# AdrianoEttari/DiffusionRemoteSensing

Hardware: AMD Instinct MI355X
Metric: unet_denoise_steps_per_s (higher is better)
Workload: dtype f16 main + block-scaled fp6 (e2m3) cross terms of tap pairs on the wide 3x3 layers (FL, 11 of 11 launches of the dominant kernel); split bf16 x3 (hi + lo) everywhere else; f32 accumulate

## Files before the change

### diffusionremotesensing_amd/_lib.py

```python
import ctypes as C
import os

_HERE = os.path.dirname(os.path.abspath(__file__))
LIB_PATH = os.path.join(_HERE, "libdrs_hip.so")

IMPL_DIRECT, IMPL_MFMA_F32, IMPL_MFMA_BF16X3, IMPL_MFMA_F16 = 0, 1, 2, 3
IMPL_BY_NAME = {"direct": IMPL_DIRECT, "mfma_f32": IMPL_MFMA_F32, "mfma_bf16x3": IMPL_MFMA_BF16X3,
                "mfma_f16": IMPL_MFMA_F16}
FWD_REUSE_COND = 1
PLAN_KEEP_ALL = 1
PLAN_TRAIN = 2
VARIANT_SUPERRES, VARIANT_SAR_TO_NDVI, VARIANT_GENERATION = 0, 1, 2


class UNetConfig(C.Structure):
    _fields_ = [("batch", C.c_int), ("lr_batch", C.c_int), ("image_channels", C.c_int), ("out_dim", C.c_int),
                ("height", C.c_int), ("width", C.c_int), ("magnification", C.c_int), ("impl", C.c_int),
                ("bn_eps", C.c_float), ("flags", C.c_int), ("variant", C.c_int),
                ("cond_channels", C.c_int), ("num_classes", C.c_int)]


_P, _I, _L, _Z, _F = C.c_void_p, C.c_int, C.c_int64, C.c_size_t, C.c_float
SIGNATURES = {
    "drs_last_error": (C.c_char_p, []),
    "drs_abi_version": (_I, []),
    "drs_noise_images": (_I, [_P, _P, _P, _P, _I, _P, _I, _L, _P]),
    "drs_sampler_step": (_I, [_P, _P, _P, _I, _P, _P, _P, _I, _L, _P]),
    "drs_sampler_step_cfg": (_I, [_P, _P, _P, C.c_float, _P, _I, _P, _P, _P, _I, C.c_int64, _P]),
    "drs_ddim_step": (_I, [_P, _P, _P, C.c_float, _P, _I, _I, C.c_float, _P, _I, C.c_int64, _P]),
    "drs_inpaint_step": (_I, [_P, _P, _P, _F, _P, _P, _P] + [_I] * 8 + [_F, _P, _P, _P, _I, _P]),
    "drs_renoise": (_I, [_P, _P, _I, _I, _P, _I, _L, _P]),
    "drs_adam_multi": (_I, [_P, _I, C.c_int64, C.c_double, C.c_double, C.c_double, C.c_double, _P]),
    "drs_ema_multi": (_I, [_P, _I, C.c_int64, C.c_double, _I, _P]),
    "drs_downblur_scratch_bytes": (_Z, [_I, _I, _I, _I, _I, _I]),
    "drs_downblur_u8": (_I, [_P, _I, _I, _I, _I, _I, _I, C.c_float, _P, _P, _P, _Z, _P]),
    "drs_add_noise_clip_f32": (_I, [_P, _P, _I, _I, _I, _I, _P]),
    "drs_gather_pairs_f32": (_I, [_P, _P, _P, _I, _L, _I, _I, _P, _P, _P]),
    "drs_gather_u8_f32": (_I, [_P, _P, _P, _I, _L, _I, _P, _P, _P]),
    "drs_aggregate_tiles": (_I, [_P, _P, _P, _P, _P, _I, _I, _I, _I, _I, _P]),
    "drs_gather_tiles": (_I, [_P, _P, _P, _I, _I, _I, _I, _I, _I, _I, _P]),
    "drs_blend_step": (_I, [_P] * 6 + [_I] * 6 + [_P, _P, _P, _I, _P]),
    "drs_blend_step_ddim": (_I, [_P] * 6 + [_I] * 7 + [_F, _P, _I, _P]),
    "drs_metrics_workspace_bytes": (_Z, [_I] * 4),
    "drs_metrics_pointwise": (_I, [_P, _P, _P] + [_I] * 5 + [_P, _Z, _P]),
    "drs_ssim": (_I, [_P, _P, _P] + [_I] * 5 + [_P, _Z, _P]),
    "drs_conv2d_workspace_bytes": (_Z, [_I] * 11),
    "drs_conv2d_nchw": (_I, [_P, _P, _P, _P] + [_I] * 12 + [_P, _Z, _I, _P]),
    "drs_upconv_fused_workspace_bytes": (_Z, [_I] * 5),
    "drs_upconv_fused_nchw": (_I, [_P] * 9 + [_I] + [_P, _P] + [_I] * 5 + [_P, _Z, _P]),
    "drs_bicubic_upsample_nchw": (_I, [_P, _P, _I, _I, _I, _I, _I, _P]),
    "drs_time_mlp": (_I, [_P] * 7 + [_I, _I, _I, _P]),
    "drs_unet_plan_create": (_I, [C.POINTER(_P), C.POINTER(UNetConfig)]),
    "drs_unet_plan_destroy": (None, [_P]),
    "drs_unet_num_params": (_I, [_P]),
    "drs_unet_param_name": (C.c_char_p, [_P, _I]),
    "drs_unet_param_numel": (_L, [_P, _I]),
    "drs_unet_packed_bytes": (_Z, [_P]),
    "drs_unet_workspace_bytes": (_Z, [_P]),
    "drs_unet_pack_weights": (_I, [_P, C.POINTER(_P), C.POINTER(_F), _P, _Z, _P]),
    "drs_unet_forward": (_I, [_P, _P, _P, _P, _P, _P, _P, _Z, _I, _P]),
    "drs_unet_forward_labels": (_I, [_P, _P, _P, _P, _P, _P, _I, _P, _P, _Z, _I, _P]),
    "drs_unet_num_tensors": (_I, [_P]),
    "drs_unet_tensor_name": (C.c_char_p, [_P, _I]),
    "drs_unet_tensor_shape": (_I, [_P, _I] + [C.POINTER(_I)] * 4),
    "drs_unet_read_tensor": (_I, [_P, _I, _P, _P, _P]),
    "drs_unet_packed_bwd_bytes": (_Z, [_P]),
    "drs_unet_backward": (_I, [_P, _P, _P, _Z, _P, _P, _P, C.POINTER(_P), _P, _Z, _P]),
    "drs_unet_backward_labels": (_I, [_P, _P, _P, _Z, _P, _P, _P, _I, _P, C.POINTER(_P), _P, _Z, _P]),
    "drs_unet_check_faults": (_I, [_P, _P, _P]),
    "drs_unet_profile_enable": (_I, [_P, _I]),
    "drs_unet_profile_num_ops": (_I, [_P]),
    "drs_unet_profile_read": (_I, [_P, _I, C.c_char_p, _I, C.POINTER(_F), C.POINTER(C.c_double), C.POINTER(C.c_double)]),
    "drs_unet_profile_num_launches": (_I, [_P]),
    "drs_unet_profile_launch": (_I, [_P, _I, C.c_char_p, _I, C.c_char_p, _I]),
    "drs_vgg_plan_create": (_I, [C.POINTER(_P), _I, _I, _I, _I]),
    "drs_vgg_plan_destroy": (None, [_P]),
    "drs_vgg_packed_bytes": (_Z, [_P]),
    "drs_vgg_workspace_bytes": (_Z, [_P]),
    "drs_vgg_pack_weights": (_I, [_P, C.POINTER(_P), _P, _Z, _P]),
    "drs_vgg_forward": (_I, [_P, _P, _P, _P, _P, _I, _P, _Z, _P]),
    "drs_vgg_backward": (_I, [_P, _P, _P, _P, _P, _Z, _P]),
    "drs_vgg_profile_enable": (_I, [_P, _I]),
    "drs_vgg_profile_num_ops": (_I, [_P]),
    "drs_vgg_profile_read": (_I, [_P, _I, C.c_char_p, _I, C.POINTER(_F), C.POINTER(C.c_double)]),
}

_lib = None


def lib_path():
    return os.environ.get("DRS_LIB", LIB_PATH)


def load():
    global _lib
    if _lib is not None:
        return _lib
    path = lib_path()
    if not os.path.exists(path):
        raise RuntimeError(
            f"{path} not found: the HIP kernels are not built. Run `python -c 'import __graft_entry__ as g; "
            "g.build()'` (needs hipcc, cross-compiles for gfx950 without a GPU). There is no CPU fallback.")
    lib = C.CDLL(path)
    for name, (res, args) in SIGNATURES.items():
        fn = getattr(lib, name)
        fn.restype = res
        fn.argtypes = args
    _lib = lib
    return lib


class RangeFault(RuntimeError):
    """DRS_ERR_RANGE from drs_unet_check_faults: an activation left fp16's range in the FL arithmetic; the plan has switched
    itself to the split-bf16 kernels, the forwards since the last check must be run again."""


def check(status, what):
    if status != 0:
# ... 6 lines not shown
```

### diffusionremotesensing_amd/csrc/resblock0_sp.hip

```cpp
#include <stdio.h>
#include <stdlib.h>

#include "conv_epilogue.h"
#include "mfma_policy.h"
#include "sp_sync.h"

namespace {

constexpr int TW_ = 16, TH_ = 8, IW = TW_ + 2, IH = TH_ + 2, NPIX = IW * IH, NBLK_A = (NPIX + 15) / 16;
constexpr int IMG1 = 5 * 4 * 64 * 16, IMG2 = 36 * 32 * 16, IMGS = 4 * 32 * 16, WIN = NPIX * 128;
constexpr int NPOST = 16;
constexpr int XPLANE = (TH_ + 4) * (TW_ + 4) * 16 + 64, XT = 4 * XPLANE;

#ifdef DRS_SP_TIMELINE
__device__ unsigned long long drs_rb0_tl[32];
#define RB_STAMP(i) do { const unsigned long long t_ = __builtin_amdgcn_s_memtime(); tl[i] += t_ - tl_last; tl_last = t_; } while (0)
#else
#define RB_STAMP(i) do { } while (0)
#endif

__global__ __launch_bounds__(512, 1) void resblock0_kernel(ResBlock0Desc d, unsigned w1_gimage, unsigned w2_gimage,
                                                           unsigned ws_gimage, int debug) {
  extern __shared__ __attribute__((aligned(16))) char smem[];
  using P = PolicyBF16X3;
  using Frag = typename P::Frag;
  auto mfma = [](const bf16x8& w, const bf16x8& x, const f32x4& c) __attribute__((always_inline)) {
    return __builtin_amdgcn_mfma_f32_16x16x32_bf16(w, x, c, 0, 0, 0);
  };
  const int tid = threadIdx.x, lane = tid & 63, wave = __builtin_amdgcn_readfirstlane(tid >> 6);
  const int lr = lane & 15, kg = lane >> 4;
  char* sW1 = smem;
  char* sW2 = sW1 + 2 * IMG1;
  char* sWs = sW2 + 2 * IMG2;
  char* sWinAll = sWs + 2 * IMGS;
  char* sXAll = sWinAll + 2 * WIN;
  float* sB1 = reinterpret_cast<float*>(sXAll + 2 * XT);
  float* sB2 = sB1 + 64;
  unsigned* sCntRaw = reinterpret_cast<unsigned*>(sB2 + 32);
  float* sPost = sB2 + 32 + 8;
  const int npost = min(d.N, NPOST);
  {
    const char* w1 = reinterpret_cast<const char*>(d.w1);
    for (int i = tid; i < 2 * 20 * 64; i += 512) {
      const int im = i >= 20 * 64, idx = im ? i - 20 * 64 : i;
      const int ch = idx % 64, kgp = (idx / 64) & 3, j = idx / (4 * 64), tap = 2 * j + (kgp >> 1);
      u32x4 v = {0u, 0u, 0u, 0u};
      if (tap < 9) v = *reinterpret_cast<const u32x4*>(w1 + (size_t)im * w1_gimage + ((size_t)(tap * 4 + (kgp & 1)) * 64 + ch) * 16);
      *reinterpret_cast<u32x4*>(sW1 + (size_t)im * IMG1 + (size_t)idx * 16) = v;
    }
    auto copy = [&](char* dst, const char* src, int bytes) __attribute__((always_inline)) {
      for (int o = tid * 16; o < bytes; o += 512 * 16) *reinterpret_cast<u32x4*>(dst + o) = *reinterpret_cast<const u32x4*>(src + o);
    };
    const char* w2 = reinterpret_cast<const char*>(d.w2);
    const char* wsc = reinterpret_cast<const char*>(d.ws);
    copy(sW2, w2, IMG2);
    copy(sW2 + IMG2, w2 + w2_gimage, IMG2);
    copy(sWs, wsc, IMGS);
    copy(sWs + IMGS, wsc + ws_gimage, IMGS);
    for (int i = tid; i < 64; i += 512) sB1[i] = d.b1[i];
    for (int i = tid; i < 32; i += 512) sB2[i] = d.b2[i] + d.bs[i];
    if (tid < 8) sCntRaw[tid] = 0u;
    for (int i = tid; i < npost * 32; i += 512) sPost[i] = d.temb[(size_t)(i >> 5) * d.temb_cs + (i & 31)];
  }
  __syncthreads();

  const int grp = wave >> 2, gw = wave & 3;
  char* sWin = sWinAll + grp * WIN;
  const sp_flag_ptr cWritten = (sp_flag_ptr)(sCntRaw + 2 * grp), cRead = (sp_flag_ptr)(sCntRaw + 2 * grp + 1);
  const int gx = d.W / TW_, gy = d.H / TH_;
  const int total = d.N * gy * gx;
  const int xcd = blockIdx.x & 7, member = blockIdx.x >> 3, members = gridDim.x >> 3;
  const int t_lo = (int)((long long)total * xcd / 8), t_hi = (int)((long long)total * (xcd + 1) / 8);
  const char* zero = reinterpret_cast<const char*>(d.zero_line);
  const char* xb = reinterpret_cast<const char*>(d.x);
  char* sX = sXAll + grp * XT;
  const sp_flag_ptr cTile = (sp_flag_ptr)(sCntRaw + 4 + grp);
  constexpr int XPIX = (TH_ + 4) * (TW_ + 4), XW = TW_ + 4;
  int tx0 = 0, ty0 = 0, n = 0;
  const int qstep_ = 2 * (int)(gridDim.x >> 3);
  const int step_x = qstep_ % gx, step_y = (qstep_ / gx) % gy, step_n = qstep_ / (gx * gy);
  int bx = 0, by = 0;
  auto place_first = [&](int q) __attribute__((always_inline)) {
    bx = q % gx; by = (q / gx) % gy; n = q / (gx * gy);
    tx0 = bx * TW_; ty0 = by * TH_;
  };
  auto place_next = [&]() __attribute__((always_inline)) {
    bx += step_x;
    if (bx >= gx) { bx -= gx; ++by; }
    by += step_y;
    if (by >= gy) { by -= gy; ++n; }
    n += step_n;
    tx0 = bx * TW_; ty0 = by * TH_;
  };
  unsigned goff[4];
#pragma unroll
  for (int i = 0; i < 4; ++i) {
    const int e = i * 256 + gw * 64 + lane, pix = min(e >> 2, XPIX - 1);
    const int py = (pix * 3277) >> 16, px = pix - py * XW;
    goff[i] = (unsigned)((py * d.W + px) * 64 + (e & 3) * 16);
  }
  u32x4 xr[4];
  auto tile_load = [&]() __attribute__((always_inline)) {
    const char* ximg = xb + (size_t)n * d.H * d.W * 64;
    if (ty0 >= 2 && ty0 + TH_ + 2 <= d.H && tx0 >= 2 && tx0 + TW_ + 2 <= d.W) {
      typedef const __attribute__((address_space(1))) char* gptr;
      const unsigned long long gi = (unsigned long long)(ximg + ((long long)(ty0 - 2) * d.W + (tx0 - 2)) * 64);
      gptr g = (gptr)(((unsigned long long)(unsigned)__builtin_amdgcn_readfirstlane((int)(gi >> 32)) << 32) |
                      (unsigned)__builtin_amdgcn_readfirstlane((int)(unsigned)gi));
      asm volatile("" : "+s"(g));
#pragma unroll
      for (int i = 0; i < 4; ++i) xr[i] = *(const __attribute__((address_space(1))) u32x4*)(g + goff[i]);
    } else {
#pragma unroll
      for (int i = 0; i < 4; ++i) {
        const int e = i * 256 + gw * 64 + lane, pix = e >> 2;
        const int py = (pix * 3277) >> 16, px = pix - py * XW;
        const int y = ty0 - 2 + py, x = tx0 - 2 + px;
        const bool ok = pix < XPIX && y >= 0 && y < d.H && x >= 0 && x < d.W;
        xr[i] = *reinterpret_cast<const u32x4*>(ok ? ximg + ((size_t)y * d.W + x) * 64 + (e & 3) * 16 : zero);
      }
    }
  };
  auto tile_store = [&]() __attribute__((always_inline)) {
#pragma unroll
    for (int i = 0; i < 4; ++i) {
      const int e = i * 256 + gw * 64 + lane;
      if ((e >> 2) < XPIX) *reinterpret_cast<u32x4*>(sX + (e & 3) * XPLANE + (e >> 2) * 16) = xr[i];
    }
    sp_release(cTile, lane);
  };
  constexpr int MAXB = NBLK_A / 4;
  static_assert(MAXB * 4 == NBLK_A, "three blocks per wave");
  int wp[MAXB], relL[MAXB], tapL[5];
#pragma unroll
  for (int b = 0; b < MAXB; ++b) {
    const int p = min((gw + 4 * b) * 16 + lr, NPIX - 1);
    const int py = (p * 3641) >> 16, px = p - py * IW;
    wp[b] = p;
    relL[b] = ((py + 1) * XW + px + 1) * 16 + (kg & 1) * XPLANE;
  }
#pragma unroll
  for (int j = 0; j < 5; ++j) {
    const int tap = min(2 * j + (kg >> 1), 8);
    tapL[j] = ((tap / 3 - 1) * XW + tap % 3 - 1) * 16;
  }
  auto operand = [&](int b, int j) __attribute__((always_inline)) {
    const char* p = sX + relL[b] + tapL[j];
    return Frag{*reinterpret_cast<const bf16x8*>(p), *reinterpret_cast<const bf16x8*>(p + 2 * XPLANE)};
  };
  const int q0 = t_lo + 2 * member + grp, qstep = 2 * members;
#ifdef DRS_SP_TIMELINE
  unsigned long long tl[8] = {0, 0, 0, 0, 0, 0, 0, 0};
  const unsigned long long tl_begin = __builtin_amdgcn_s_memtime();
  unsigned long long tl_last = tl_begin, tl_n = 0;
  if ((debug & 1) && grp == 1) return;
#endif
  if (q0 < t_hi) {
    place_first(q0);
    tile_load();
    tile_store();
    if (q0 + qstep < t_hi) {
      place_next();
      tile_load();
      asm volatile("" :: "v"(xr[0]), "v"(xr[1]), "v"(xr[2]), "v"(xr[3]));
    }
  }
  if (grp == 1) { __builtin_amdgcn_s_sleep(64); __builtin_amdgcn_s_sleep(32); }
  unsigned k = 0;
  u32x4 kept[4] = {};
  int cbx = q0 % gx, cby = (q0 / gx) % gy, cn = q0 / (gx * gy);
  for (int q = q0; q < t_hi; q += qstep, ++k) {
#ifdef DRS_SP_TIMELINE
    ++tl_n;
#endif
    RB_STAMP(7);
    const int cty0 = cby * TH_, ctx0 = cbx * TW_;
    sp_poll_lds(cTile, 4u * (k + 1), d.fault);
    const bool more = q + qstep < t_hi;
    f32x4 acc[MAXB][4];
#pragma unroll
    for (int b = 0; b < MAXB; ++b)
#pragma unroll
      for (int t = 0; t < 4; ++t) acc[b][t] = f32x4{0.f, 0.f, 0.f, 0.f};
    const char* w1lane = sW1 + ((size_t)kg * 64 + lr) * 16;
    Frag a[2][MAXB], wfa[2][2];
#pragma unroll
    for (int b = 0; b < MAXB; ++b) a[0][b] = operand(b, 0);
#pragma unroll
    for (int u = 0; u < 2; ++u) wfa[0][u] = P::load(w1lane, (size_t)IMG1, (size_t)(u * 16) * 16);
#pragma unroll
    for (int st = 0; st < 10; ++st) {
      const int j = st >> 1, h = st & 1;
      if (st + 1 < 10) {
#pragma unroll
        for (int u = 0; u < 2; ++u)
          wfa[(st + 1) & 1][u] = P::load(w1lane, (size_t)IMG1, (size_t)(((st + 1) >> 1) * 4 * 64 + (((st + 1) & 1) * 2 + u) * 16) * 16);
      }
      if (h == 0 && j + 1 < 5) {
#pragma unroll
        for (int b = 0; b < MAXB; ++b) a[(j + 1) & 1][b] = operand(b, j + 1);
      }
      {
        const Frag (&wf)[2] = wfa[st & 1];
#pragma unroll
        for (int u = 0; u < 2; ++u)
#pragma unroll
          for (int b = 0; b < MAXB; ++b) acc[b][2 * h + u] = mfma(wf[u].lo, a[j & 1][b].hi, acc[b][2 * h + u]);
#pragma unroll
        for (int u = 0; u < 2; ++u)
#pragma unroll
          for (int b = 0; b < MAXB; ++b) acc[b][2 * h + u] = mfma(wf[u].hi, a[j & 1][b].lo, acc[b][2 * h + u]);
#pragma unroll
        for (int u = 0; u < 2; ++u)
#pragma unroll
          for (int b = 0; b < MAXB; ++b) acc[b][2 * h + u] = mfma(wf[u].hi, a[j & 1][b].hi, acc[b][2 * h + u]);
      }
      if (h == 0 && j + 1 < 5) __builtin_amdgcn_sched_group_barrier(0x100, 4 + 2 * MAXB, 0);
      else if (st + 1 < 10) __builtin_amdgcn_sched_group_barrier(0x100, 4, 0);
      __builtin_amdgcn_sched_group_barrier(0x008, 18, 0);
      __builtin_amdgcn_sched_barrier(0);
    }
    asm volatile("" :: "v"(kept[0]), "v"(kept[1]), "v"(kept[2]), "v"(kept[3]));
    RB_STAMP(0);
    Frag xs[2];
#pragma unroll
    for (int r = 0; r < 2; ++r) {
      const char* p = sX + ((2 + 2 * gw + r) * XW + 2 + lr) * 16 + (kg & 1) * XPLANE;
      xs[r] = Frag{*reinterpret_cast<const bf16x8*>(p), *reinterpret_cast<const bf16x8*>(p + 2 * XPLANE)};
    }
    float bm[8], bs[8], te[8];
    {
      const float4 m0 = *reinterpret_cast<const float4*>(sB1 + kg * 8), m1 = *reinterpret_cast<const float4*>(sB1 + kg * 8 + 4);
      const float4 s0 = *reinterpret_cast<const float4*>(sB1 + 32 + kg * 8), s1 = *reinterpret_cast<const float4*>(sB1 + 32 + kg * 8 + 4);
      float4 e0, e1;
      if (cn < npost) {
        e0 = *reinterpret_cast<const float4*>(sPost + cn * 32 + kg * 8); e1 = *reinterpret_cast<const float4*>(sPost + cn * 32 + kg * 8 + 4);
      } else {
        const float* gp = d.temb + (size_t)cn * d.temb_cs + kg * 8;
        e0 = *reinterpret_cast<const float4*>(gp); e1 = *reinterpret_cast<const float4*>(gp + 4);
      }
      bm[0] = m0.x; bm[1] = m0.y; bm[2] = m0.z; bm[3] = m0.w; bm[4] = m1.x; bm[5] = m1.y; bm[6] = m1.z; bm[7] = m1.w;
      bs[0] = s0.x; bs[1] = s0.y; bs[2] = s0.z; bs[3] = s0.w; bs[4] = s1.x; bs[5] = s1.y; bs[6] = s1.z; bs[7] = s1.w;
      te[0] = e0.x; te[1] = e0.y; te[2] = e0.z; te[3] = e0.w; te[4] = e1.x; te[5] = e1.y; te[6] = e1.z; te[7] = e1.w;
    }
    RB_STAMP(1);
    sp_poll_lds(cRead, 4u * k, d.fault);
    RB_STAMP(2);
#pragma unroll
    for (int b = 0; b < MAXB; ++b) {
      float v[8];
#pragma unroll
      for (int t = 0; t < 2; ++t)
#pragma unroll
        for (int i = 0; i < 4; ++i)
          v[t * 4 + i] = (drs_maxf(acc[b][t][i] + bm[t * 4 + i], 0.f) + (acc[b][t + 2][i] + bs[t * 4 + i])) + te[t * 4 + i];
      u32x4 hh, hl;
      drs_sp_split8(v, hh, hl);
      int p = wp[b];
      asm volatile("" : "+v"(p));
      const int py = (p * 3641) >> 16, px = p - py * IW;
      const int y = cty0 - 1 + py, x = ctx0 - 1 + px;
      const bool inside = y >= 0 && y < d.H && x >= 0 && x < d.W;
      if (!inside) { hh = u32x4{0u, 0u, 0u, 0u}; hl = u32x4{0u, 0u, 0u, 0u}; }
      if ((gw + 4 * b) * 16 + lr < NPIX) {
        char* wpix = sWin + p * 128;
        const int s0 = ((kg + p) & 7) * 16;
        *reinterpret_cast<u32x4*>(wpix + s0) = hh;
        *reinterpret_cast<u32x4*>(wpix + (s0 ^ 64)) = hl;
      }
    }
    sp_release(cWritten, lane);
    sp_poll_lds(cWritten, 4u * (k + 1), d.fault);
    if (more) tile_store();
    RB_STAMP(3);
    f32x4 o[2][2];
#pragma unroll
    for (int r = 0; r < 2; ++r)
#pragma unroll
      for (int t = 0; t < 2; ++t) o[r][t] = f32x4{0.f, 0.f, 0.f, 0.f};
    const char* w2lane = sW2 + ((size_t)kg * 32 + lr) * 16;
    auto win = [&](int row, int kx) __attribute__((always_inline)) {
      const int p = (2 * gw + row) * IW + lr + kx;
      const char* wpix = sWin + p * 128;
      const int s0 = ((kg + p) & 7) * 16;
      return Frag{*reinterpret_cast<const bf16x8*>(wpix + s0), *reinterpret_cast<const bf16x8*>(wpix + (s0 ^ 64))};
    };
    Frag wr_[4][3];
    auto win_row = [&](int row) __attribute__((always_inline)) {
#pragma unroll
      for (int kx = 0; kx < 3; ++kx) wr_[row][kx] = win(row, kx);
    };
    win_row(0);
    win_row(1);
    {
      const char* wslane = sWs + ((size_t)kg * 32 + lr) * 16;
      Frag wfb[2][2];
      wfb[0][0] = P::load(w2lane, (size_t)IMG2, 0);
      wfb[0][1] = P::load(w2lane, (size_t)IMG2, (size_t)16 * 16);
#pragma unroll
      for (int st = 0; st < 10; ++st) {
#pragma unroll
        for (int t = 0; t < 2; ++t) {
          if (st + 1 < 9) wfb[(st + 1) & 1][t] = P::load(w2lane, (size_t)IMG2, (size_t)((st + 1) * 4 * 32 + t * 16) * 16);
          else if (st + 1 < 10) wfb[(st + 1) & 1][t] = P::load(wslane, (size_t)IMGS, (size_t)(t * 16) * 16);
        }
        if (st == 0) win_row(2);
        if (st == 3) {
          win_row(3);
          sp_release(cRead, lane);
        }
        const int ky = st < 9 ? st / 3 : 0, kx = st < 9 ? st % 3 : 0;
        const Frag& x0f = st < 9 ? wr_[ky][kx] : xs[0];
        const Frag& x1f = st < 9 ? wr_[ky + 1][kx] : xs[1];
        const Frag (&wf)[2] = wfb[st & 1];
#pragma unroll
        for (int t = 0; t < 2; ++t) { o[0][t] = mfma(wf[t].lo, x0f.hi, o[0][t]); o[1][t] = mfma(wf[t].lo, x1f.hi, o[1][t]); }
#pragma unroll
        for (int t = 0; t < 2; ++t) { o[0][t] = mfma(wf[t].hi, x0f.lo, o[0][t]); o[1][t] = mfma(wf[t].hi, x1f.lo, o[1][t]); }
#pragma unroll
        for (int t = 0; t < 2; ++t) { o[0][t] = mfma(wf[t].hi, x0f.hi, o[0][t]); o[1][t] = mfma(wf[t].hi, x1f.hi, o[1][t]); }
        if (st == 0 || st == 3) __builtin_amdgcn_sched_group_barrier(0x100, 10, 0);
        else if (st + 1 < 10) __builtin_amdgcn_sched_group_barrier(0x100, 4, 0);
        __builtin_amdgcn_sched_group_barrier(0x008, 12, 0);
        __builtin_amdgcn_sched_barrier(0);
      }
    }
    if (q + 2 * qstep < t_hi) {
      place_next();
      tile_load();
    }
    RB_STAMP(4);
    {
      const float4 b0 = *reinterpret_cast<const float4*>(sB2 + kg * 8), b1 = *reinterpret_cast<const float4*>(sB2 + kg * 8 + 4);
      const float bb[8] = {b0.x, b0.y, b0.z, b0.w, b1.x, b1.y, b1.z, b1.w};
      const bool lo = lr < 8;
      const size_t pix0 = ((size_t)cn * d.H + cty0 + 2 * gw) * d.W + ctx0 + (lr & 7);
      char* g = reinterpret_cast<char*>(d.out) + pix0 * 128 + (lo ? 0 : 64) + kg * 16;
#pragma unroll
      for (int r = 0; r < 2; ++r) {
        float v[8];
#pragma unroll
        for (int i = 0; i < 4; ++i) { v[i] = drs_maxf(o[r][0][i] + bb[i], 0.f); v[4 + i] = drs_maxf(o[r][1][i] + bb[4 + i], 0.f); }
        u32x4 H, L;
        drs_sp_split8(v, H, L);
        const u32x4 got = drs_dpp_swap8(lo ? L : H);
        kept[2 * r] = lo ? H : got;
        kept[2 * r + 1] = lo ? got : L;
        char* gr = g + (size_t)r * d.W * 128;
        drs_store16(gr, kept[2 * r]);
        drs_store16(gr + 8 * 128, kept[2 * r + 1]);
      }
    }
    RB_STAMP(5);
    cbx += step_x;
    if (cbx >= gx) { cbx -= gx; ++cby; }
    cby += step_y;
    if (cby >= gy) { cby -= gy; ++cn; }
    cn += step_n;
  }
#ifdef DRS_SP_TIMELINE
  if (blockIdx.x == 0 && (wave == 0 || wave == 7) && lane == 0) {
    const int o = wave == 0 ? 0 : 16;
    for (int i = 0; i < 8; ++i) drs_rb0_tl[o + i] = tl[i];
    drs_rb0_tl[o + 8] = tl_n;
    drs_rb0_tl[o + 9] = __builtin_amdgcn_s_memtime() - tl_begin;
  }
#endif
}

size_t resblock0_lds(int N) { return (size_t)2 * (IMG1 + IMG2 + IMGS) + 2 * WIN + 2 * XT + (size_t)(64 + 32 + 8 + 32 * (N < NPOST ? N : NPOST)) * 4; }

}

bool drs_resblock0_supported(int Cin, int Cout, int H, int W) {
  static const bool env = !(getenv("DRS_RB0") && atoi(getenv("DRS_RB0")) == 0);
  return env && Cin == 16 && Cout == 32 && H >= 32 && W >= 32 && H % TH_ == 0 && W % TW_ == 0;
}

int drs_launch_resblock0(const ResBlock0Desc& d, hipStream_t s) {
  DRS_REQUIRE(drs_resblock0_supported(16, 32, d.H, d.W), DRS_ERR_SHAPE, "resblock0: H=%d W=%d", d.H, d.W);
  DRS_REQUIRE(d.x && d.w1 && d.b1 && d.temb && d.w2 && d.b2 && d.ws && d.bs && d.out && d.zero_line, DRS_ERR_ARG, "resblock0: null pointer");
  if (d.N == 0) return DRS_OK;
  int num_cu = 0;
  {
    const int rc = drs_kernel_prepare(reinterpret_cast<const void*>(resblock0_kernel), 160 * 1024, &num_cu);
    if (rc) return rc;
  }
  const unsigned w1_gimage = 9u * 4u * 64u * 16u, w2_gimage = 9u * 4u * 32u * 16u, ws_gimage = 4u * 32u * 16u;
  const int blocks = num_cu / 8 * 8;
  DRS_LAUNCH(resblock0_kernel, dim3((unsigned)blocks), dim3(512), resblock0_lds(d.N), s, d, w1_gimage, w2_gimage, ws_gimage, 0);
  DRS_CHECK_HIP(hipGetLastError());
#ifdef DRS_SP_TIMELINE
  {
    unsigned long long h[32];
    const int dbg = getenv("DRS_RB0_DEBUG") ? atoi(getenv("DRS_RB0_DEBUG")) : 0;
    hipEvent_t e0, e1;
    float ms = 0.f;
    DRS_CHECK_HIP(hipEventCreate(&e0)); DRS_CHECK_HIP(hipEventCreate(&e1));
    DRS_CHECK_HIP(hipEventRecord(e0, s));
    DRS_LAUNCH(resblock0_kernel, dim3((unsigned)blocks), dim3(512), resblock0_lds(d.N), s, d, w1_gimage, w2_gimage, ws_gimage, dbg);
    DRS_CHECK_HIP(hipEventRecord(e1, s));
    DRS_CHECK_HIP(hipStreamSynchronize(s));
    DRS_CHECK_HIP(hipEventElapsedTime(&ms, e0, e1));
    (void)hipEventDestroy(e0); (void)hipEventDestroy(e1);
    DRS_CHECK_HIP(hipMemcpyFromSymbol(h, HIP_SYMBOL(drs_rb0_tl), sizeof(h)));
    for (int w = 0; w < 2; ++w) {
      const unsigned long long* t = h + 16 * w;
      const double sc = t[8] ? 1.0 / (double)t[8] : 0.0;
      fprintf(stderr, "resblock0 %dx%d wave %d: %.1f us, %llu patches, alive %llu ticks (%.0f / patch) | top %.0f  A-mfma %.0f  A-epi %.0f  bar1 %.0f  "
              "winstore+bar2 %.0f  B-mfma %.0f  B-epi %.0f\n", d.H, d.W, w ? 7 : 0, ms * 1e3, t[8], t[9], t[9] * sc, t[7] * sc, t[0] * sc, t[1] * sc,
              t[2] * sc, t[3] * sc, t[4] * sc, t[5] * sc);
    }
  }
#endif
  return DRS_OK;
}
```

### include/drs_hip.h

```cpp
#ifndef DRS_HIP_H
#define DRS_HIP_H

#include <stddef.h>
#include <stdint.h>

#ifdef __cplusplus
extern "C" {
#endif

#define DRS_API __attribute__((visibility("default")))

typedef void* drs_stream_t;
typedef struct drs_plan drs_plan;

enum {
  DRS_OK = 0,
  DRS_ERR_ARG = 1,
  DRS_ERR_SHAPE = 2,
  DRS_ERR_HIP = 3,
  DRS_ERR_WORKSPACE = 4,
  DRS_ERR_STATE = 5,
  DRS_ERR_RANGE = 6
};

// ... 96 lines not shown
                          drs_stream_t stream);

DRS_API int drs_bicubic_upsample_nchw(const float* x, float* y, int N, int C, int H, int W, int scale,
                              drs_stream_t stream);

DRS_API int drs_time_mlp(const int64_t* t, const float* inv_freq, const float* W1, const float* b1, const float* W2,
                 const float* b2, float* out, int B, int dim_in, int dim_out, drs_stream_t stream);


typedef struct drs_unet_config {
  int batch;
  int lr_batch;
  int image_channels;
  int out_dim;
  int height, width;
  int magnification;
  int impl;
  float bn_eps;
  int flags;
  int variant;
  int cond_channels;
  int num_classes;
} drs_unet_config;
#define DRS_VARIANT_SUPERRES 0
#define DRS_VARIANT_SAR_TO_NDVI 1
#define DRS_VARIANT_GENERATION 2
#define DRS_PLAN_KEEP_ALL 1
#define DRS_PLAN_TRAIN 2

DRS_API int drs_unet_plan_create(drs_plan** plan, const drs_unet_config* cfg);
DRS_API void drs_unet_plan_destroy(drs_plan* plan);

DRS_API int drs_unet_num_params(const drs_plan* plan);
DRS_API const char* drs_unet_param_name(const drs_plan* plan, int i);
DRS_API int64_t drs_unet_param_numel(const drs_plan* plan, int i);

DRS_API size_t drs_unet_packed_bytes(const drs_plan* plan);
DRS_API size_t drs_unet_workspace_bytes(const drs_plan* plan);

DRS_API int drs_unet_pack_weights(drs_plan* plan, const void* const* params, const float* inv_freq_host, void* packed,
                          size_t packed_bytes, drs_stream_t stream);

#define DRS_FWD_REUSE_COND 1
DRS_API int drs_unet_forward(drs_plan* plan, const void* packed, const float* x, const int64_t* t, const float* lr_img,
                     float* out, void* workspace, size_t workspace_bytes, int flags, drs_stream_t stream);
DRS_API int drs_unet_forward_labels(drs_plan* plan, const void* packed, const float* x, const int64_t* t, const float* cond,
                            const int64_t* labels, int label_batch, float* out, void* workspace,
                            size_t workspace_bytes, int flags, drs_stream_t stream);

DRS_API int drs_unet_num_tensors(const drs_plan* plan);
DRS_API const char* drs_unet_tensor_name(const drs_plan* plan, int i);
DRS_API int drs_unet_tensor_shape(const drs_plan* plan, int i, int* n, int* c, int* h, int* w);
DRS_API int drs_unet_read_tensor(const drs_plan* plan, int i, const void* workspace, float* dst_nchw, drs_stream_t stream);

DRS_API size_t drs_unet_packed_bwd_bytes(const drs_plan* plan);
DRS_API int drs_unet_backward(drs_plan* plan, const void* packed, void* packed_bwd, size_t packed_bwd_bytes, const float* x,
                      const int64_t* t, const float* dout, float* const* grads, void* workspace, size_t workspace_bytes,
                      drs_stream_t stream);
DRS_API int drs_unet_backward_labels(drs_plan* plan, const void* packed, void* packed_bwd, size_t packed_bwd_bytes,
                             const float* x, const int64_t* t, const int64_t* labels, int label_batch,
                             const float* dout, float* const* grads, void* workspace, size_t workspace_bytes,
                             drs_stream_t stream);

DRS_API int drs_unet_check_faults(drs_plan* plan, const void* packed, drs_stream_t stream);

DRS_API int drs_unet_profile_enable(drs_plan* plan, int on);
DRS_API int drs_unet_profile_num_ops(const drs_plan* plan);
DRS_API int drs_unet_profile_read(drs_plan* plan, int i, char* name, int name_len, float* ms, double* flops, double* bytes);
DRS_API int drs_unet_profile_num_launches(const drs_plan* plan);
DRS_API int drs_unet_profile_launch(const drs_plan* plan, int i, char* op, int op_len, char* kernel, int kernel_len);

typedef struct drs_vgg_plan drs_vgg_plan;
DRS_API int drs_vgg_plan_create(drs_vgg_plan** plan, int batch, int height, int width, int impl);
DRS_API void drs_vgg_plan_destroy(drs_vgg_plan* plan);
DRS_API size_t drs_vgg_packed_bytes(const drs_vgg_plan* plan);
DRS_API size_t drs_vgg_workspace_bytes(const drs_vgg_plan* plan);
DRS_API int drs_vgg_pack_weights(drs_vgg_plan* plan, const void* const* params, void* packed, size_t packed_bytes,
                         drs_stream_t stream);
DRS_API int drs_vgg_forward(drs_vgg_plan* plan, const void* packed, const float* pred, const float* target, float* loss,
                    int save, void* workspace, size_t workspace_bytes, drs_stream_t stream);
DRS_API int drs_vgg_backward(drs_vgg_plan* plan, const void* packed, const float* grad_loss, float* dpred, void* workspace,
                     size_t workspace_bytes, drs_stream_t stream);
DRS_API int drs_vgg_profile_enable(drs_vgg_plan* plan, int on);
DRS_API int drs_vgg_profile_num_ops(const drs_vgg_plan* plan);
DRS_API int drs_vgg_profile_read(drs_vgg_plan* plan, int i, char* name, int name_len, float* ms, double* flops);

#ifdef __cplusplus
}
#endif
#endif
```

Before: 825.3.

## Walk resblock0 tiles in vertical strips, reusing overlapping halo rows of conv1 output

The resblock0 fused kernel now assigns each workgroup a vertical strip of several 16x8 patches instead of independent patches. After the first patch of a strip, it loads only the new input rows, carries the overlapping input halo in LDS, and reuses the last two rows of the first conv's output window. Phase A therefore computes fewer MFMA blocks per non-first patch, using a half-block split across waves. A host helper picks the strip height so there are still enough strips to fill the GPU. The trade-off is more control-flow variants and less parallel granularity.

After: 826.4, median of 4. About the same (+0.1%).

```diff
diff --git a/diffusionremotesensing_amd/_lib.py b/diffusionremotesensing_amd/_lib.py
--- a/diffusionremotesensing_amd/_lib.py
+++ b/diffusionremotesensing_amd/_lib.py
@@ -64,6 +64,7 @@
     "drs_unet_tensor_name": (C.c_char_p, [_P, _I]),
     "drs_unet_tensor_shape": (_I, [_P, _I] + [C.POINTER(_I)] * 4),
     "drs_unet_read_tensor": (_I, [_P, _I, _P, _P, _P]),
+    "drs_resblock0_strip_rows": (_I, [_I] * 4),
     "drs_unet_packed_bwd_bytes": (_Z, [_P]),
     "drs_unet_backward": (_I, [_P, _P, _P, _Z, _P, _P, _P, C.POINTER(_P), _P, _Z, _P]),
     "drs_unet_backward_labels": (_I, [_P, _P, _P, _Z, _P, _P, _P, _I, _P, C.POINTER(_P), _P, _Z, _P]),
diff --git a/diffusionremotesensing_amd/csrc/resblock0_sp.hip b/diffusionremotesensing_amd/csrc/resblock0_sp.hip
--- a/diffusionremotesensing_amd/csrc/resblock0_sp.hip
+++ b/diffusionremotesensing_amd/csrc/resblock0_sp.hip
@@ -1,5 +1,7 @@
 #include <stdio.h>
 #include <stdlib.h>
+
+#include <type_traits>
 
 #include "conv_epilogue.h"
 #include "mfma_policy.h"
@@ -7,7 +9,7 @@
 
 namespace {
 
-constexpr int TW_ = 16, TH_ = 8, IW = TW_ + 2, IH = TH_ + 2, NPIX = IW * IH, NBLK_A = (NPIX + 15) / 16;
+constexpr int TW_ = 16, TH_ = 8, IW = TW_ + 2, IH = TH_ + 2, NPIX = IW * IH;
 constexpr int IMG1 = 5 * 4 * 64 * 16, IMG2 = 36 * 32 * 16, IMGS = 4 * 32 * 16, WIN = NPIX * 128;
 constexpr int NPOST = 16;
 constexpr int XPLANE = (TH_ + 4) * (TW_ + 4) * 16 + 64, XT = 4 * XPLANE;
@@ -20,7 +22,7 @@
 #endif
 
 __global__ __launch_bounds__(512, 1) void resblock0_kernel(ResBlock0Desc d, unsigned w1_gimage, unsigned w2_gimage,
-                                                           unsigned ws_gimage, int debug) {
+                                                           unsigned ws_gimage, int strip_patches, int debug) {
   extern __shared__ __attribute__((aligned(16))) char smem[];
   using P = PolicyBF16X3;
   using Frag = typename P::Frag;
@@ -67,7 +69,8 @@
   const int grp = wave >> 2, gw = wave & 3;
   char* sWin = sWinAll + grp * WIN;
   const sp_flag_ptr cWritten = (sp_flag_ptr)(sCntRaw + 2 * grp), cRead = (sp_flag_ptr)(sCntRaw + 2 * grp + 1);
-  const int gx = d.W / TW_, gy = d.H / TH_;
+  const int SP = strip_patches, R = SP * TH_;
+  const int gx = d.W / TW_, gy = d.H / R;
   const int total = d.N * gy * gx;
   const int xcd = blockIdx.x & 7, member = blockIdx.x >> 3, members = gridDim.x >> 3;
   const int t_lo = (int)((long long)total * xcd / 8), t_hi = (int)((long long)total * (xcd + 1) / 8);
@@ -75,154 +78,231 @@
   const char* xb = reinterpret_cast<const char*>(d.x);
   char* sX = sXAll + grp * XT;
   const sp_flag_ptr cTile = (sp_flag_ptr)(sCntRaw + 4 + grp);
-  constexpr int XPIX = (TH_ + 4) * (TW_ + 4), XW = TW_ + 4;
-  int tx0 = 0, ty0 = 0, n = 0;
+  constexpr int XPIX = (TH_ + 4) * (TW_ + 4), XW = TW_ + 4, XNEW = TH_ * XW, XCARRY = TH_ * XW * 16;
   const int qstep_ = 2 * (int)(gridDim.x >> 3);
   const int step_x = qstep_ % gx, step_y = (qstep_ / gx) % gy, step_n = qstep_ / (gx * gy);
-  int bx = 0, by = 0;
+  int bx = 0, by = 0, n = 0, pj = 0;
+  int tx0 = 0, ty0 = 0;
   auto place_first = [&](int q) __attribute__((always_inline)) {
-    bx = q % gx; by = (q / gx) % gy; n = q / (gx * gy);
-    tx0 = bx * TW_; ty0 = by * TH_;
+    bx = q % gx; by = (q / gx) % gy; n = q / (gx * gy); pj = 0;
+    tx0 = bx * TW_; ty0 = by * R;
   };
   auto place_next = [&]() __attribute__((always_inline)) {
-    bx += step_x;
-    if (bx >= gx) { bx -= gx; ++by; }
-    by += step_y;
-    if (by >= gy) { by -= gy; ++n; }
-    n += step_n;
-    tx0 = bx * TW_; ty0 = by * TH_;
-  };
-  unsigned goff[4];
-#pragma unroll
-  for (int i = 0; i < 4; ++i) {
-    const int e = i * 256 + gw * 64 + lane, pix = min(e >> 2, XPIX - 1);
+    if (++pj == SP) {
+      pj = 0;
+      bx += step_x;
+      if (bx >= gx) { bx -= gx; ++by; }
+      by += step_y;
+      if (by >= gy) { by -= gy; ++n; }
+      n += step_n;
+    }
+    tx0 = bx * TW_; ty0 = by * R + pj * TH_;
+  };
+  auto goff = [&](int i, int npix) __attribute__((always_inline)) {
+    int l_ = lane;
+    asm volatile("" : "+v"(l_));
+    const int e = i * 256 + gw * 64 + l_, pix = min(e >> 2, npix - 1);
     const int py = (pix * 3277) >> 16, px = pix - py * XW;
-    goff[i] = (unsigned)((py * d.W + px) * 64 + (e & 3) * 16);
-  }
+    return (unsigned)((py * d.W + px) * 64 + (e & 3) * 16);
+  };
   u32x4 xr[4];
+  bool xr_whole = true;
   auto tile_load = [&]() __attribute__((always_inline)) {
     const char* ximg = xb + (size_t)n * d.H * d.W * 64;
-    if (ty0 >= 2 && ty0 + TH_ + 2 <= d.H && tx0 >= 2 && tx0 + TW_ + 2 <= d.W) {
-      typedef const __attribute__((address_space(1))) char* gptr;
-      const unsigned long long gi = (unsigned long long)(ximg + ((long long)(ty0 - 2) * d.W + (tx0 - 2)) * 64);
-      gptr g = (gptr)(((unsigned long long)(unsigned)__builtin_amdgcn_readfirstlane((int)(gi >> 32)) << 32) |
-                      (unsigned)__builtin_amdgcn_readfirstlane((int)(unsigned)gi));
-      asm volatile("" : "+s"(g));
-#pragma unroll
-      for (int i = 0; i < 4; ++i) xr[i] = *(const __attribute__((address_space(1))) u32x4*)(g + goff[i]);
+    typedef const __attribute__((address_space(1))) char* gptr;
+    xr_whole = pj == 0;
+    if (xr_whole) {
+      if (ty0 >= 2 && ty0 + TH_ + 2 <= d.H && tx0 >= 2 && tx0 + TW_ + 2 <= d.W) {
+        const unsigned long long gi = (unsigned long long)(ximg + ((long long)(ty0 - 2) * d.W + (tx0 - 2)) * 64);
+        gptr g = (gptr)(((unsigned long long)(unsigned)__builtin_amdgcn_readfirstlane((int)(gi >> 32)) << 32) |
+                        (unsigned)__builtin_amdgcn_readfirstlane((int)(unsigned)gi));
+        asm volatile("" : "+s"(g));
+#pragma unroll
+        for (int i = 0; i < 4; ++i) xr[i] = *(const __attribute__((address_space(1))) u32x4*)(g + goff(i, XPIX));
+      } else {
+#pragma unroll
+        for (int i = 0; i < 4; ++i) {
+          const int e = i * 256 + gw * 64 + lane, pix = e >> 2;
+          const int py = (pix * 3277) >> 16, px = pix - py * XW;
+          const int y = ty0 - 2 + py, x = tx0 - 2 + px;
+          const bool ok = pix < XPIX && y >= 0 && y < d.H && x >= 0 && x < d.W;
+          xr[i] = *reinterpret_cast<const u32x4*>(ok ? ximg + ((size_t)y * d.W + x) * 64 + (e & 3) * 16 : zero);
+        }
+      }
     } else {
+      if (ty0 + TH_ + 2 <= d.H && tx0 >= 2 && tx0 + TW_ + 2 <= d.W) {
+        const unsigned long long gi = (unsigned long long)(ximg + ((long long)(ty0 + 2) * d.W + (tx0 - 2)) * 64);
+        gptr g = (gptr)(((unsigned long long)(unsigned)__builtin_amdgcn_readfirstlane((int)(gi >> 32)) << 32) |
+                        (unsigned)__builtin_amdgcn_readfirstlane((int)(unsigned)gi));
+        asm volatile("" : "+s"(g));
+#pragma unroll
+        for (int i = 0; i < 3; ++i)
+          if (i < 2 || gw < 2) xr[i] = *(const __attribute__((address_space(1))) u32x4*)(g + goff(i, XNEW));
+      } else {
+#pragma unroll
+        for (int i = 0; i < 3; ++i) {
+          const int e = i * 256 + gw * 64 + lane, pix = e >> 2;
+          const int py = (pix * 3277) >> 16, px = pix - py * XW;
+          const int y = ty0 + 2 + py, x = tx0 - 2 + px;
+          const bool ok = pix < XNEW && y < d.H && x >= 0 && x < d.W;
+          xr[i] = *reinterpret_cast<const u32x4*>(ok ? ximg + ((size_t)y * d.W + x) * 64 + (e & 3) * 16 : zero);
+        }
+      }
+    }
+  };
+  u32x4 xc[2] = {};
+  const bool xcp1 = gw == 3 && lane >= 32, xcp2 = gw < 2;
+  auto xnew_addr = [&](int i) __attribute__((always_inline)) {
+    int l_ = lane;
+    asm volatile("" : "+v"(l_));
+    const int e = i * 256 + gw * 64 + l_;
+    return sX + (e & 3) * XPLANE + ((e >> 2) + 4 * XW) * 16;
+  };
+  auto tile_carry_read = [&]() __attribute__((always_inline)) {
+    if (xcp1) xc[0] = *reinterpret_cast<const u32x4*>(xnew_addr(1));
+    if (xcp2) xc[1] = *reinterpret_cast<const u32x4*>(xnew_addr(2));
+  };
+  auto tile_store = [&]() __attribute__((always_inline)) {
+    if (xr_whole) {
 #pragma unroll
       for (int i = 0; i < 4; ++i) {
-        const int e = i * 256 + gw * 64 + lane, pix = e >> 2;
-        const int py = (pix * 3277) >> 16, px = pix - py * XW;
-        const int y = ty0 - 2 + py, x = tx0 - 2 + px;
-        const bool ok = pix < XPIX && y >= 0 && y < d.H && x >= 0 && x < d.W;
-        xr[i] = *reinterpret_cast<const u32x4*>(ok ? ximg + ((size_t)y * d.W + x) * 64 + (e & 3) * 16 : zero);
-      }
-    }
-  };
-  auto tile_store = [&]() __attribute__((always_inline)) {
-#pragma unroll
-    for (int i = 0; i < 4; ++i) {
-      const int e = i * 256 + gw * 64 + lane;
-      if ((e >> 2) < XPIX) *reinterpret_cast<u32x4*>(sX + (e & 3) * XPLANE + (e >> 2) * 16) = xr[i];
+        const int e = i * 256 + gw * 64 + lane;
+        if ((e >> 2) < XPIX) *reinterpret_cast<u32x4*>(sX + (e & 3) * XPLANE + (e >> 2) * 16) = xr[i];
+      }
+    } else {
+      if (xcp1) *reinterpret_cast<u32x4*>(xnew_addr(1) - XCARRY) = xc[0];
+      if (xcp2) *reinterpret_cast<u32x4*>(xnew_addr(2) - XCARRY) = xc[1];
+#pragma unroll
+      for (int i = 0; i < 3; ++i)
+        if (i < 2 || gw < 2) *reinterpret_cast<u32x4*>(xnew_addr(i)) = xr[i];
     }
     sp_release(cTile, lane);
   };
-  constexpr int MAXB = NBLK_A / 4;
-  static_assert(MAXB * 4 == NBLK_A, "three blocks per wave");
-  int wp[MAXB], relL[MAXB], tapL[5];
-#pragma unroll
-  for (int b = 0; b < MAXB; ++b) {
-    const int p = min((gw + 4 * b) * 16 + lr, NPIX - 1);
-    const int py = (p * 3641) >> 16, px = p - py * IW;
-    wp[b] = p;
-    relL[b] = ((py + 1) * XW + px + 1) * 16 + (kg & 1) * XPLANE;
-  }
+  int tapL[5];
 #pragma unroll
   for (int j = 0; j < 5; ++j) {
     const int tap = min(2 * j + (kg >> 1), 8);
     tapL[j] = ((tap / 3 - 1) * XW + tap % 3 - 1) * 16;
   }
-  auto operand = [&](int b, int j) __attribute__((always_inline)) {
-    const char* p = sX + relL[b] + tapL[j];
+  auto operand = [&](int rel, int j) __attribute__((always_inline)) {
+    const char* p = sX + rel + tapL[j];
     return Frag{*reinterpret_cast<const bf16x8*>(p), *reinterpret_cast<const bf16x8*>(p + 2 * XPLANE)};
   };
   const int q0 = t_lo + 2 * member + grp, qstep = 2 * members;
+  const int npatch = q0 < t_hi ? ((t_hi - q0 + qstep - 1) / qstep) * SP : 0;
 #ifdef DRS_SP_TIMELINE
   unsigned long long tl[8] = {0, 0, 0, 0, 0, 0, 0, 0};
   const unsigned long long tl_begin = __builtin_amdgcn_s_memtime();
-  unsigned long long tl_last = tl_begin, tl_n = 0;
+  unsigned long long tl_last = tl_begin, tl_n = 0, tl_first = 0;
   if ((debug & 1) && grp == 1) return;
 #endif
-  if (q0 < t_hi) {
+  if (npatch > 0) {
     place_first(q0);
     tile_load();
     tile_store();
-    if (q0 + qstep < t_hi) {
+    if (npatch > 1) {
       place_next();
       tile_load();
       asm volatile("" :: "v"(xr[0]), "v"(xr[1]), "v"(xr[2]), "v"(xr[3]));
     }
   }
   if (grp == 1) { __builtin_amdgcn_s_sleep(64); __builtin_amdgcn_s_sleep(32); }
+  u32x4 kept[4] = {};
+  int cbx = q0 % gx, cby = (q0 / gx) % gy, cn = q0 / (gx * gy), cpj = 0;
+  int cty0 = 0, ctx0 = 0;
   unsigned k = 0;
-  u32x4 kept[4] = {};
-  int cbx = q0 % gx, cby = (q0 / gx) % gy, cn = q0 / (gx * gy);
-  for (int q = q0; q < t_hi; q += qstep, ++k) {
-#ifdef DRS_SP_TIMELINE
-    ++tl_n;
-#endif
-    RB_STAMP(7);
-    const int cty0 = cby * TH_, ctx0 = cbx * TW_;
-    sp_poll_lds(cTile, 4u * (k + 1), d.fault);
-    const bool more = q + qstep < t_hi;
-    f32x4 acc[MAXB][4];
-#pragma unroll
-    for (int b = 0; b < MAXB; ++b)
+  bool more = false;
+  const char* w1lane = sW1 + ((size_t)kg * 64 + lr) * 16;
+  Frag xs[2];
+
+  auto phase_a = [&](auto mode_) __attribute__((always_inline)) {
+    constexpr int M = decltype(mode_)::value;
+    constexpr int NF = M == 0 ? 3 : 2;
+    constexpr bool HALF = M == 1 || M == 2;
+    constexpr int HC = M == 2 ? 1 : 0, NB = NF + (HALF ? 1 : 0);
+    int wp[NB], rel[NB];
+    int lr_ = lr;
+    asm volatile("" : "+v"(lr_));
+#pragma unroll
+    for (int b = 0; b < NB; ++b) {
+      const int blk = M == 0 ? gw + 4 * b : (b < 2 ? 2 * gw + b : 8);
+      const int p = M == 0 ? min(blk * 16 + lr_, NPIX - 1) : 2 * IW + blk * 16 + lr_;
+      const int py = (p * 3641) >> 16, px = p - py * IW;
+      wp[b] = p;
+      rel[b] = ((py + 1) * XW + px + 1) * 16 + (kg & 1) * XPLANE;
+    }
+    f32x4 acc[NF][4], acch[2];
+#pragma unroll
+    for (int b = 0; b < NF; ++b)
 #pragma unroll
       for (int t = 0; t < 4; ++t) acc[b][t] = f32x4{0.f, 0.f, 0.f, 0.f};
-    const char* w1lane = sW1 + ((size_t)kg * 64 + lr) * 16;
-    Frag a[2][MAXB], wfa[2][2];
-#pragma unroll
-    for (int b = 0; b < MAXB; ++b) a[0][b] = operand(b, 0);
-#pragma unroll
-    for (int u = 0; u < 2; ++u) wfa[0][u] = P::load(w1lane, (size_t)IMG1, (size_t)(u * 16) * 16);
-#pragma unroll
-    for (int st = 0; st < 10; ++st) {
-      const int j = st >> 1, h = st & 1;
-      if (st + 1 < 10) {
-#pragma unroll
-        for (int u = 0; u < 2; ++u)
-          wfa[(st + 1) & 1][u] = P::load(w1lane, (size_t)IMG1, (size_t)(((st + 1) >> 1) * 4 * 64 + (((st + 1) & 1) * 2 + u) * 16) * 16);
-      }
-      if (h == 0 && j + 1 < 5) {
-#pragma unroll
-        for (int b = 0; b < MAXB; ++b) a[(j + 1) & 1][b] = operand(b, j + 1);
-      }
-      {
-        const Frag (&wf)[2] = wfa[st & 1];
-#pragma unroll
-        for (int u = 0; u < 2; ++u)
-#pragma unroll
-          for (int b = 0; b < MAXB; ++b) acc[b][2 * h + u] = mfma(wf[u].lo, a[j & 1][b].hi, acc[b][2 * h + u]);
-#pragma unroll
-        for (int u = 0; u < 2; ++u)
-#pragma unroll
-          for (int b = 0; b < MAXB; ++b) acc[b][2 * h + u] = mfma(wf[u].hi, a[j & 1][b].lo, acc[b][2 * h + u]);
-#pragma unroll
-        for (int u = 0; u < 2; ++u)
-#pragma unroll
-          for (int b = 0; b < MAXB; ++b) acc[b][2 * h + u] = mfma(wf[u].hi, a[j & 1][b].hi, acc[b][2 * h + u]);
-      }
-      if (h == 0 && j + 1 < 5) __builtin_amdgcn_sched_group_barrier(0x100, 4 + 2 * MAXB, 0);
-      else if (st + 1 < 10) __builtin_amdgcn_sched_group_barrier(0x100, 4, 0);
-      __builtin_amdgcn_sched_group_barrier(0x008, 18, 0);
+    acch[0] = acch[1] = f32x4{0.f, 0.f, 0.f, 0.f};
+    Frag a[2][NB];
+    bf16x8 wlo[4], whi[4];
+    auto wload = [&](int j, int t, int image) __attribute__((always_inline)) {
+      return *reinterpret_cast<const bf16x8*>(w1lane + (size_t)image * IMG1 + (size_t)(j * 4 * 64 + t * 16) * 16);
+    };
+    constexpr int NCH = 4 * NF + (HALF ? 2 : 0);
+#pragma unroll
+    for (int b = 0; b < NB; ++b) a[0][b] = operand(rel[b], 0);
+#pragma unroll
+    for (int t = 0; t < 4; ++t) wlo[t] = wload(0, t, 1);
+#pragma unroll
+    for (int j = 0; j < 5; ++j) {
+      const Frag (&af)[NB] = a[j & 1];
+#pragma unroll
+      for (int t = 0; t < 4; ++t) whi[t] = wload(j, t, 0);
+#pragma unroll
+      for (int t = 0; t < 4; ++t)
+#pragma unroll
+        for (int b = 0; b < NF; ++b) acc[b][t] = mfma(wlo[t], af[b].hi, acc[b][t]);
+      if constexpr (HALF) { acch[0] = mfma(wlo[HC], af[NB - 1].hi, acch[0]); acch[1] = mfma(wlo[HC + 2], af[NB - 1].hi, acch[1]); }
+      __builtin_amdgcn_sched_group_barrier(0x100, 4, 0);
+      __builtin_amdgcn_sched_group_barrier(0x008, NCH, 0);
+      __builtin_amdgcn_sched_barrier(0);
+      if (j + 1 < 5) {
+#pragma unroll
+        for (int t = 0; t < 4; ++t) wlo[t] = wload(j + 1, t, 1);
+#pragma unroll
+        for (int b = 0; b < NB; ++b) a[(j + 1) & 1][b] = operand(rel[b], j + 1);
+      }
+#pragma unroll
+      for (int t = 0; t < 4; ++t)
+#pragma unroll
+        for (int b = 0; b < NF; ++b) acc[b][t] = mfma(whi[t], af[b].lo, acc[b][t]);
+      if constexpr (HALF) { acch[0] = mfma(whi[HC], af[NB - 1].lo, acch[0]); acch[1] = mfma(whi[HC + 2], af[NB - 1].lo, acch[1]); }
+      if (j + 1 < 5) __builtin_amdgcn_sched_group_barrier(0x100, 4 + 2 * NB, 0);
+      __builtin_amdgcn_sched_group_barrier(0x008, NCH, 0);
+      __builtin_amdgcn_sched_barrier(0);
+#pragma unroll
+      for (int t = 0; t < 4; ++t)
+#pragma unroll
+        for (int b = 0; b < NF; ++b) acc[b][t] = mfma(whi[t], af[b].hi, acc[b][t]);
+      if constexpr (HALF) { acch[0] = mfma(whi[HC], af[NB - 1].hi, acch[0]); acch[1] = mfma(whi[HC + 2], af[NB - 1].hi, acch[1]); }
+      __builtin_amdgcn_sched_group_barrier(0x008, NCH, 0);
       __builtin_amdgcn_sched_barrier(0);
     }
     asm volatile("" :: "v"(kept[0]), "v"(kept[1]), "v"(kept[2]), "v"(kept[3]));
     RB_STAMP(0);
-    Frag xs[2];
+    u32x4 oh[2] = {}, ol[2] = {};
+    uint2 ohh = {0u, 0u}, olh = {0u, 0u};
+    if constexpr (M != 0) {
+#pragma unroll
+      for (int b = 0; b < NF; ++b)
+        if (wp[b] >= (IH - 2) * IW) {
+          const char* wpix = sWin + wp[b] * 128;
+          const int s0 = ((kg + wp[b]) & 7) * 16;
+          oh[b] = *reinterpret_cast<const u32x4*>(wpix + s0);
+          ol[b] = *reinterpret_cast<const u32x4*>(wpix + (s0 ^ 64));
+        }
+      if constexpr (HALF) {
+        const char* wpix = sWin + wp[NB - 1] * 128;
+        const int s0 = ((kg + wp[NB - 1]) & 7) * 16 + HC * 8;
+        ohh = *reinterpret_cast<const uint2*>(wpix + s0);
+        olh = *reinterpret_cast<const uint2*>(wpix + (s0 ^ 64));
+      }
+    }
+    if (more && !xr_whole) tile_carry_read();
 #pragma unroll
     for (int r = 0; r < 2; ++r) {
       const char* p = sX + ((2 + 2 * gw + r) * XW + 2 + lr) * 16 + (kg & 1) * XPLANE;
@@ -246,8 +326,29 @@
     RB_STAMP(1);
     sp_poll_lds(cRead, 4u * k, d.fault);
     RB_STAMP(2);
-#pragma unroll
-    for (int b = 0; b < MAXB; ++b) {
+    if constexpr (M != 0) {
+#pragma unroll
+      for (int b = 0; b < NF; ++b)
+        if (wp[b] >= (IH - 2) * IW) {
+          char* wpix = sWin + (wp[b] - (IH - 2) * IW) * 128;
+          const int s0 = ((kg + wp[b]) & 7) * 16;
+          *reinterpret_cast<u32x4*>(wpix + s0) = oh[b];
+          *reinterpret_cast<u32x4*>(wpix + (s0 ^ 64)) = ol[b];
+        }
+      if constexpr (HALF) {
+        char* wpix = sWin + (wp[NB - 1] - (IH - 2) * IW) * 128;
+        const int s0 = ((kg + wp[NB - 1]) & 7) * 16 + HC * 8;
+        *reinterpret_cast<uint2*>(wpix + s0) = ohh;
+        *reinterpret_cast<uint2*>(wpix + (s0 ^ 64)) = olh;
+      }
+    }
+    auto outside = [&](int p) __attribute__((always_inline)) {
+      const int py = (p * 3641) >> 16, px = p - py * IW;
+      const int y = cty0 - 1 + py, x = ctx0 - 1 + px;
+      return !(y >= 0 && y < d.H && x >= 0 && x < d.W);
+    };
+#pragma unroll
+    for (int b = 0; b < NF; ++b) {
       float v[8];
 #pragma unroll
       for (int t = 0; t < 2; ++t)
@@ -258,21 +359,48 @@
       drs_sp_split8(v, hh, hl);
       int p = wp[b];
       asm volatile("" : "+v"(p));
-      const int py = (p * 3641) >> 16, px = p - py * IW;
-      const int y = cty0 - 1 + py, x = ctx0 - 1 + px;
-      const bool inside = y >= 0 && y < d.H && x >= 0 && x < d.W;
-      if (!inside) { hh = u32x4{0u, 0u, 0u, 0u}; hl = u32x4{0u, 0u, 0u, 0u}; }
-      if ((gw + 4 * b) * 16 + lr < NPIX) {
+      if (outside(p)) { hh = u32x4{0u, 0u, 0u, 0u}; hl = u32x4{0u, 0u, 0u, 0u}; }
+      if (M != 0 || (gw + 4 * b) * 16 + lr < NPIX) {
         char* wpix = sWin + p * 128;
         const int s0 = ((kg + p) & 7) * 16;
         *reinterpret_cast<u32x4*>(wpix + s0) = hh;
         *reinterpret_cast<u32x4*>(wpix + (s0 ^ 64)) = hl;
       }
     }
+    if constexpr (HALF) {
+      float v[4];
+#pragma unroll
+      for (int i = 0; i < 4; ++i)
+        v[i] = (drs_maxf(acch[0][i] + bm[HC * 4 + i], 0.f) + (acch[1][i] + bs[HC * 4 + i])) + te[HC * 4 + i];
+      unsigned hh[2], hl[2];
+      drs_sp_split4(v, hh, hl);
+      int p = wp[NB - 1];
+      asm volatile("" : "+v"(p));
+      if (outside(p)) { hh[0] = hh[1] = 0u; hl[0] = hl[1] = 0u; }
+      char* wpix = sWin + p * 128;
+      const int s0 = ((kg + p) & 7) * 16 + HC * 8;
+      *reinterpret_cast<uint2*>(wpix + s0) = uint2{hh[0], hh[1]};
+      *reinterpret_cast<uint2*>(wpix + (s0 ^ 64)) = uint2{hl[0], hl[1]};
+    }
     sp_release(cWritten, lane);
     sp_poll_lds(cWritten, 4u * (k + 1), d.fault);
     if (more) tile_store();
     RB_STAMP(3);
+  };
+
+  for (int it = 0; it < npatch; ++it, ++k) {
+#ifdef DRS_SP_TIMELINE
+    ++tl_n;
+    if (cpj == 0) ++tl_first;
+#endif
+    RB_STAMP(7);
+    cty0 = cby * R + cpj * TH_; ctx0 = cbx * TW_;
+    sp_poll_lds(cTile, 4u * (k + 1), d.fault);
+    more = it + 1 < npatch;
+    if (cpj == 0) phase_a(std::integral_constant<int, 0>{});
+    else if (gw == 0) phase_a(std::integral_constant<int, 1>{});
+    else if (gw == 1) phase_a(std::integral_constant<int, 2>{});
+    else phase_a(std::integral_constant<int, 3>{});
     f32x4 o[2][2];
 #pragma unroll
     for (int r = 0; r < 2; ++r)
@@ -325,7 +453,7 @@
         __builtin_amdgcn_sched_barrier(0);
       }
     }
-    if (q + 2 * qstep < t_hi) {
+    if (it + 2 < npatch) {
       place_next();
       tile_load();
     }
@@ -352,11 +480,14 @@
       }
     }
     RB_STAMP(5);
-    cbx += step_x;
-    if (cbx >= gx) { cbx -= gx; ++cby; }
-    cby += step_y;
-    if (cby >= gy) { cby -= gy; ++cn; }
-    cn += step_n;
+    if (++cpj == SP) {
+      cpj = 0;
+      cbx += step_x;
+      if (cbx >= gx) { cbx -= gx; ++cby; }
+      cby += step_y;
+      if (cby >= gy) { cby -= gy; ++cn; }
+      cn += step_n;
+    }
   }
 #ifdef DRS_SP_TIMELINE
   if (blockIdx.x == 0 && (wave == 0 || wave == 7) && lane == 0) {
@@ -364,6 +495,7 @@
     for (int i = 0; i < 8; ++i) drs_rb0_tl[o + i] = tl[i];
     drs_rb0_tl[o + 8] = tl_n;
     drs_rb0_tl[o + 9] = __builtin_amdgcn_s_memtime() - tl_begin;
+    drs_rb0_tl[o + 10] = tl_first;
   }
 #endif
 }
@@ -375,6 +507,14 @@
 bool drs_resblock0_supported(int Cin, int Cout, int H, int W) {
   static const bool env = !(getenv("DRS_RB0") && atoi(getenv("DRS_RB0")) == 0);
   return env && Cin == 16 && Cout == 32 && H >= 32 && W >= 32 && H % TH_ == 0 && W % TW_ == 0;
+}
+
+extern "C" int drs_resblock0_strip_rows(int N, int H, int W, int num_cu) {
+  if (N <= 0 || H < TH_ || W < TW_ || H % TH_ || W % TW_ || num_cu < 8) return 0;
+  const long long groups = 2LL * (num_cu / 8 * 8), cols = (long long)N * (W / TW_);
+  for (int r = H; r >= TH_; r -= TH_)
+    if (H % r == 0 && cols * (H / r) >= groups) return r;
+  return H;
 }
 
 int drs_launch_resblock0(const ResBlock0Desc& d, hipStream_t s) {
@@ -388,7 +528,8 @@
   }
   const unsigned w1_gimage = 9u * 4u * 64u * 16u, w2_gimage = 9u * 4u * 32u * 16u, ws_gimage = 4u * 32u * 16u;
   const int blocks = num_cu / 8 * 8;
-  DRS_LAUNCH(resblock0_kernel, dim3((unsigned)blocks), dim3(512), resblock0_lds(d.N), s, d, w1_gimage, w2_gimage, ws_gimage, 0);
+  const int strip_patches = drs_resblock0_strip_rows(d.N, d.H, d.W, num_cu) / TH_;
+  DRS_LAUNCH(resblock0_kernel, dim3((unsigned)blocks), dim3(512), resblock0_lds(d.N), s, d, w1_gimage, w2_gimage, ws_gimage, strip_patches, 0);
   DRS_CHECK_HIP(hipGetLastError());
 #ifdef DRS_SP_TIMELINE
   {
@@ -398,7 +539,7 @@
     float ms = 0.f;
     DRS_CHECK_HIP(hipEventCreate(&e0)); DRS_CHECK_HIP(hipEventCreate(&e1));
     DRS_CHECK_HIP(hipEventRecord(e0, s));
-    DRS_LAUNCH(resblock0_kernel, dim3((unsigned)blocks), dim3(512), resblock0_lds(d.N), s, d, w1_gimage, w2_gimage, ws_gimage, dbg);
+    DRS_LAUNCH(resblock0_kernel, dim3((unsigned)blocks), dim3(512), resblock0_lds(d.N), s, d, w1_gimage, w2_gimage, ws_gimage, strip_patches, dbg);
     DRS_CHECK_HIP(hipEventRecord(e1, s));
     DRS_CHECK_HIP(hipStreamSynchronize(s));
     DRS_CHECK_HIP(hipEventElapsedTime(&ms, e0, e1));
@@ -407,8 +548,8 @@
     for (int w = 0; w < 2; ++w) {
       const unsigned long long* t = h + 16 * w;
       const double sc = t[8] ? 1.0 / (double)t[8] : 0.0;
-      fprintf(stderr, "resblock0 %dx%d wave %d: %.1f us, %llu patches, alive %llu ticks (%.0f / patch) | top %.0f  A-mfma %.0f  A-epi %.0f  bar1 %.0f  "
-              "winstore+bar2 %.0f  B-mfma %.0f  B-epi %.0f\n", d.H, d.W, w ? 7 : 0, ms * 1e3, t[8], t[9], t[9] * sc, t[7] * sc, t[0] * sc, t[1] * sc,
+      fprintf(stderr, "resblock0 %dx%d wave %d: %.1f us, %llu patches (%llu whole-window), alive %llu ticks (%.0f / patch) | top %.0f  A-mfma %.0f  A-epi %.0f  bar1 %.0f  "
+              "winstore+bar2 %.0f  B-mfma %.0f  B-epi %.0f\n", d.H, d.W, w ? 7 : 0, ms * 1e3, t[8], t[10], t[9], t[9] * sc, t[7] * sc, t[0] * sc, t[1] * sc,
               t[2] * sc, t[3] * sc, t[4] * sc, t[5] * sc);
     }
   }
diff --git a/include/drs_hip.h b/include/drs_hip.h
--- a/include/drs_hip.h
+++ b/include/drs_hip.h
@@ -172,6 +172,7 @@
 DRS_API const char* drs_unet_tensor_name(const drs_plan* plan, int i);
 DRS_API int drs_unet_tensor_shape(const drs_plan* plan, int i, int* n, int* c, int* h, int* w);
 DRS_API int drs_unet_read_tensor(const drs_plan* plan, int i, const void* workspace, float* dst_nchw, drs_stream_t stream);
+DRS_API int drs_resblock0_strip_rows(int N, int H, int W, int num_cu);
 
 DRS_API size_t drs_unet_packed_bwd_bytes(const drs_plan* plan);
 DRS_API int drs_unet_backward(drs_plan* plan, const void* packed, void* packed_bwd, size_t packed_bwd_bytes, const float* x,
```
